# 10XGenomics/scan-rs

Hardware: AMD Instinct MI355X
Metric: cells/sec for top-50 PCA on 1000000x33000 @3% nnz; achieved HBM GB/s vs roofline (higher is better)
Workload: dtype f64

## Files before the change

### scan-rs_amd/csrc/dense.hip

```cpp
#include "common.hpp"

#include <algorithm>

namespace scanrs {

typedef double d2 __attribute__((ext_vector_type(2)));
typedef double d4 __attribute__((ext_vector_type(4)));

constexpr uint32_t DT = 128;
constexpr uint32_t DK = 16;
constexpr uint32_t DLD = 144;

__device__ __forceinline__ void tile_mma(const double *__restrict__ As, const double *__restrict__ Bs, uint32_t wi,
                                         uint32_t wj, uint32_t li, uint32_t lk, d4 (&acc)[4][4]) {
#pragma unroll
    for (uint32_t kk = 0; kk < DK / 4; kk++) {
        const uint32_t row = (kk * 4 + lk) * DLD;
        double a[4], b[4];
#pragma unroll
        for (int t = 0; t < 4; t++) {
            a[t] = As[row + wi * 64 + t * 16 + li];
            b[t] = Bs[row + wj * 64 + t * 16 + li];
        }
#pragma unroll
        for (int mi = 0; mi < 4; mi++)
#pragma unroll
            for (int nj = 0; nj < 4; nj++) acc[mi][nj] = __builtin_amdgcn_mfma_f64_16x16x4f64(a[mi], b[nj], acc[mi][nj], 0, 0, 0);
    }
}

__global__ __launch_bounds__(256) void gram_tiled_kernel(const double *__restrict__ X, uint32_t ldx, uint32_t n,
                                                         const double *__restrict__ Y, uint32_t ldy, uint32_t m, uint64_t rows,
                                                         uint64_t rows_per_split, const uint32_t *__restrict__ tile_ij,
                                                         double *__restrict__ slab, const int *__restrict__ skip) {
    if (skip && *skip) return;
    __shared__ double As[DK * DLD];
    __shared__ double Bs[DK * DLD];
    const uint32_t tid = threadIdx.x, lane = tid & 63u, w = tid >> 6;
    const uint32_t li = lane & 15u, lk = lane >> 4, wi = w >> 1, wj = w & 1u;
    const uint32_t i0 = tile_ij[2 * blockIdx.x] * DT, j0 = tile_ij[2 * blockIdx.x + 1] * DT;
    const uint64_t r0 = (uint64_t)blockIdx.y * rows_per_split;
    const uint64_t r1 = min(rows, r0 + rows_per_split);
    d4 acc[4][4];
#pragma unroll
    for (int a = 0; a < 4; a++)
#pragma unroll
        for (int b = 0; b < 4; b++) acc[a][b] = (d4){0, 0, 0, 0};
    const uint32_t sc = lane * 2u;
    d2 xa[4], yb[4];
    auto load_block = [&](uint64_t r) {
#pragma unroll
        for (int h = 0; h < 4; h++) {
            const uint64_t gr = r + w * 4u + h;
            const bool rv = gr < r1;
            const uint32_t c = sc;
            xa[h] = (d2){0.0, 0.0};
            yb[h] = (d2){0.0, 0.0};
            if (rv) {
                const double *xr = X + gr * ldx + i0 + c;
                const double *yr = Y + gr * ldy + j0 + c;
                if (i0 + c + 1 < n)
                    xa[h] = *reinterpret_cast<const d2 *>(xr);
                else if (i0 + c < n)
                    xa[h].x = xr[0];
                if (j0 + c + 1 < m)
                    yb[h] = *reinterpret_cast<const d2 *>(yr);
                else if (j0 + c < m)
                    yb[h].x = yr[0];
            }
        }
    };
    auto store_block = [&]() {
#pragma unroll
        for (int h = 0; h < 4; h++) {
            *reinterpret_cast<d2 *>(&As[(w * 4u + h) * DLD + sc]) = xa[h];
            *reinterpret_cast<d2 *>(&Bs[(w * 4u + h) * DLD + sc]) = yb[h];
        }
    };
    if (r0 < r1) {
        load_block(r0);
        store_block();
    }
    __syncthreads();
    for (uint64_t r = r0; r < r1; r += DK) {
        const bool more = r + DK < r1;
        if (more) load_block(r + DK);
        tile_mma(As, Bs, wi, wj, li, lk, acc);
        __syncthreads();
        if (more) store_block();
        __syncthreads();
    }
    double *__restrict__ dst = slab + (size_t)blockIdx.y * n * m;
#pragma unroll
    for (int mi = 0; mi < 4; mi++)
#pragma unroll
        for (int nj = 0; nj < 4; nj++)
#pragma unroll
            for (int reg = 0; reg < 4; reg++) {
                const uint32_t row = i0 + wi * 64 + mi * 16 + lk + 4 * reg;
                const uint32_t col = j0 + wj * 64 + nj * 16 + li;
                if (row < n && col < m) dst[(size_t)row * m + col] = acc[mi][nj][reg];
            }
}

__global__ void gram_tiled_finish_kernel(const double *__restrict__ slab, uint32_t splits, uint32_t n, uint32_t m,
                                         int symmetric, double *__restrict__ C, const int *__restrict__ skip) {
    if (skip && *skip) return;
    const uint64_t e = (uint64_t)blockIdx.x * blockDim.x + threadIdx.x;
    if (e >= (uint64_t)n * m) return;
    uint32_t row = (uint32_t)(e / m), col = (uint32_t)(e % m);
    uint64_t src = e;
    if (symmetric && row / DT > col / DT) src = (uint64_t)col * m + row;
    double s = 0.0;
    for (uint32_t k = 0; k < splits; k++) s += slab[(size_t)k * n * m + src];
    C[e] = s;
}

__global__ __launch_bounds__(256) void gemm_tiled_kernel(const double *__restrict__ X, uint32_t ldx, uint32_t n,
                                                         const double *__restrict__ W, uint32_t ldw, uint32_t m, uint64_t rows,
                                                         double alpha, double beta, const double *Cin, uint32_t ldc,
                                                         double *Out, uint32_t ldo, const int *__restrict__ skip) {
    if (skip && *skip) return;
    __shared__ double As[DK * DLD];
    __shared__ double Bs[DK * DLD];
    const uint32_t tid = threadIdx.x, lane = tid & 63u, w = tid >> 6;
    const uint32_t li = lane & 15u, lk = lane >> 4, wi = w >> 1, wj = w & 1u;
    const uint64_t r0 = (uint64_t)blockIdx.x * DT;
    const uint32_t j0 = blockIdx.y * DT;
    d4 acc[4][4];
#pragma unroll
    for (int a = 0; a < 4; a++)
#pragma unroll
        for (int b = 0; b < 4; b++) acc[a][b] = (d4){0, 0, 0, 0};
    const uint32_t ai = tid >> 3, ak = (tid & 7u) * 2u;
    const uint32_t bk = tid >> 4, bc = (tid & 15u) * 8u;
    d2 av[4], bv[4];
    auto load_block = [&](uint32_t k0) {
        const uint32_t kb = k0 + bk;
        const double *wr = W + (size_t)kb * ldw + j0 + bc;
        const uint32_t kk = k0 + ak;
#pragma unroll
        for (int h = 0; h < 4; h++) {
            const uint64_t arow = r0 + ai + 32u * h;
            av[h] = (d2){0.0, 0.0};
            if (arow < rows) {
                const double *xr = X + arow * ldx + kk;
                if (kk + 1 < n)
                    av[h] = *reinterpret_cast<const d2 *>(xr);
                else if (kk < n)
                    av[h].x = xr[0];
            }
            const uint32_t c = bc + 2u * h;
            bv[h] = (d2){0.0, 0.0};
            if (kb < n) {
                if (j0 + c + 1 < m)
                    bv[h].x = wr[2 * h], bv[h].y = wr[2 * h + 1];
                else if (j0 + c < m)
                    bv[h].x = wr[2 * h];
            }
        }
    };
    auto store_block = [&]() {
#pragma unroll
        for (int h = 0; h < 4; h++) {
            As[ak * DLD + ai + 32u * h] = av[h].x;
            As[(ak + 1u) * DLD + ai + 32u * h] = av[h].y;
            *reinterpret_cast<d2 *>(&Bs[bk * DLD + bc + 2u * h]) = bv[h];
        }
    };
    if (n > 0) {
        load_block(0);
        store_block();
    }
    __syncthreads();
    for (uint32_t k0 = 0; k0 < n; k0 += DK) {
        const bool more = k0 + DK < n;
        if (more) load_block(k0 + DK);
        tile_mma(As, Bs, wi, wj, li, lk, acc);
        __syncthreads();
        if (more) store_block();
        __syncthreads();
    }
#pragma unroll
    for (int mi = 0; mi < 4; mi++)
#pragma unroll
        for (int reg = 0; reg < 4; reg++) {
            const uint64_t row = r0 + wi * 64 + mi * 16 + lk + 4 * reg;
            if (row >= rows) continue;
#pragma unroll
            for (int nj = 0; nj < 4; nj++) {
                const uint32_t col = j0 + wj * 64 + nj * 16 + li;
                if (col >= m) continue;
                double r = alpha * acc[mi][nj][reg];
                if (beta != 0.0) r = fma(beta, Cin[row * ldc + col], r);
                Out[row * ldo + col] = r;
            }
        }
}

constexpr uint32_t SK_R = 256, SK_C = 64, SK_ALD = 272, SK_BLD = 80;
__global__ __launch_bounds__(256) void gemm_skinny_kernel(const double *__restrict__ X, uint32_t ldx, uint32_t n,
                                                          const double *__restrict__ W, uint32_t ldw, uint32_t m, uint64_t rows,
                                                          double alpha, double beta, const double *Cin, uint32_t ldc,
                                                          double *Out, uint32_t ldo, const int *__restrict__ skip) {
    if (skip && *skip) return;
    __shared__ double As[DK * SK_ALD];
    __shared__ double Bs[DK * SK_BLD];
    const uint32_t tid = threadIdx.x, lane = tid & 63u, w = tid >> 6;
    const uint32_t li = lane & 15u, lk = lane >> 4;
    const uint64_t r0 = (uint64_t)blockIdx.x * SK_R;
    const uint32_t j0 = blockIdx.y * SK_C;
    d4 acc[4][4];
#pragma unroll
    for (int a = 0; a < 4; a++)
#pragma unroll
        for (int b = 0; b < 4; b++) acc[a][b] = (d4){0, 0, 0, 0};
    const uint32_t ai = tid >> 3, ak = (tid & 7u) * 2u;
    const uint32_t bk = tid >> 4, bc = (tid & 15u) * 4u;
    d2 av[8];
    double bv[4];
    auto load_block = [&](uint32_t k0) {
        const uint32_t kk = k0 + ak;
#pragma unroll
        for (int h = 0; h < 8; h++) {
            const uint64_t arow = r0 + ai + 32u * h;
            av[h] = (d2){0.0, 0.0};
            if (arow < rows) {
                const double *xr = X + arow * ldx + kk;
                if (kk + 1 < n)
                    av[h] = *reinterpret_cast<const d2 *>(xr);
                else if (kk < n)
                    av[h].x = xr[0];
            }
        }
        const uint32_t kb = k0 + bk;
        const double *wr = W + (size_t)kb * ldw + j0 + bc;
#pragma unroll
        for (int h = 0; h < 4; h++) bv[h] = (kb < n && j0 + bc + h < m) ? wr[h] : 0.0;
    };
    auto store_block = [&]() {
#pragma unroll
        for (int h = 0; h < 8; h++) {
            As[ak * SK_ALD + ai + 32u * h] = av[h].x;
            As[(ak + 1u) * SK_ALD + ai + 32u * h] = av[h].y;
        }
#pragma unroll
        for (int h = 0; h < 4; h++) Bs[bk * SK_BLD + bc + h] = bv[h];
    };
    if (n > 0) {
        load_block(0);
        store_block();
    }
    __syncthreads();
    for (uint32_t k0 = 0; k0 < n; k0 += DK) {
        const bool more = k0 + DK < n;
        if (more) load_block(k0 + DK);
#pragma unroll
        for (uint32_t kk = 0; kk < DK / 4; kk++) {
            double a[4], b[4];
#pragma unroll
            for (int t = 0; t < 4; t++) {
                a[t] = As[(kk * 4 + lk) * SK_ALD + w * 64 + t * 16 + li];
                b[t] = Bs[(kk * 4 + lk) * SK_BLD + t * 16 + li];
            }
#pragma unroll
            for (int mi = 0; mi < 4; mi++)
#pragma unroll
                for (int nj = 0; nj < 4; nj++) acc[mi][nj] = __builtin_amdgcn_mfma_f64_16x16x4f64(a[mi], b[nj], acc[mi][nj], 0, 0, 0);
        }
        __syncthreads();
        if (more) store_block();
        __syncthreads();
    }
#pragma unroll
    for (int mi = 0; mi < 4; mi++)
#pragma unroll
        for (int reg = 0; reg < 4; reg++) {
            const uint64_t row = r0 + w * 64 + mi * 16 + lk + 4 * reg;
            if (row >= rows) continue;
#pragma unroll
            for (int nj = 0; nj < 4; nj++) {
                const uint32_t col = j0 + nj * 16 + li;
                if (col >= m) continue;
                double r = alpha * acc[mi][nj][reg];
                if (beta != 0.0) r = fma(beta, Cin[row * ldc + col], r);
                Out[row * ldo + col] = r;
            }
        }
}

constexpr uint32_t CHOL_NMAX = 128;
#ifndef SCANRS_CHOL_TD
#define SCANRS_CHOL_TD 32
#endif
constexpr uint32_t CHOL_TD = SCANRS_CHOL_TD;
constexpr int CHOL_E = CHOL_NMAX / CHOL_TD;
__global__ __launch_bounds__(CHOL_TD * CHOL_TD) void chol_rinv_kernel(const double *__restrict__ G, uint32_t n, double rows, int pass, int check_only,
                                                        int *__restrict__ ctl, double *__restrict__ Rinv, double *__restrict__ info) {
    __shared__ double rowbuf[CHOL_NMAX], colbuf[CHOL_NMAX], red[3 * CHOL_TD * CHOL_TD];
    const uint32_t tid = threadIdx.x, nt = blockDim.x, ty = tid / CHOL_TD, tx = tid % CHOL_TD;
    const uint32_t wy0 = (uint32_t)__builtin_amdgcn_readfirstlane((int)(tid >> 6)) * (64u / CHOL_TD);
    auto identity_out = [&]() {
        if (check_only) return;
        for (uint32_t e = tid; e < n * n; e += nt) Rinv[e] = (e / n == e % n) ? 1.0 : 0.0;
    };
    if (ctl[0]) {
        identity_out();
        return;
    }
    double err = 0.0, dmax = 0.0;
    int bad = 0;
    for (uint32_t e = tid; e < n * n; e += nt) {
        const uint32_t i = e / n, j = e - i * n;
        const double g = G[e];
        if (!isfinite(g)) bad = 1;
        err = fmax(err, fabs(g - (i == j ? 1.0 : 0.0)));
        if (i == j) dmax = fmax(dmax, g);
    }
    red[tid] = err;
    red[nt + tid] = dmax;
    red[2 * nt + tid] = (double)bad;
    __syncthreads();
    for (uint32_t s = nt / 2; s > 0; s >>= 1) {
        if (tid < s) {
            red[tid] = fmax(red[tid], red[tid + s]);
            red[nt + tid] = fmax(red[nt + tid], red[nt + tid + s]);
            red[2 * nt + tid] = fmax(red[2 * nt + tid], red[2 * nt + tid + s]);
        }
        __syncthreads();
    }
    err = red[0];
    dmax = red[nt];
    bad = red[2 * nt] != 0.0;
    __syncthreads();
    if (tid == 0 && info) info[0] = err;
    if (bad) {
        if (tid == 0) {
            ctl[0] = 1;
            ctl[1] = 2;
        }
        identity_out();
        return;
    }
    if (pass >= 1 && err < 5e-14 * sqrt((double)n)) {
        if (tid == 0) ctl[0] = 1;
        identity_out();
        return;
    }
    if (check_only) return;
    double A[CHOL_E][CHOL_E];
    double shift = 0.0;
    for (int tries = 0;; tries++) {
#pragma unroll
        for (int a = 0; a < CHOL_E; a++)
#pragma unroll
            for (int b = 0; b < CHOL_E; b++) {
                const uint32_t i = ty + CHOL_TD * a, j = tx + CHOL_TD * b;
                A[a][b] = (i < n && j < n && j >= i) ? G[i * n + j] + (i == j ? shift : 0.0) : 0.0;
            }
        bool failed = false;
        for (uint32_t k = 0; k < n; k++) {
            const uint32_t ka = k / CHOL_TD, kt = k % CHOL_TD;
#pragma unroll
            for (int a = 0; a < CHOL_E; a++)
                if ((uint32_t)a == ka && ty == kt) {
#pragma unroll
                    for (int b = 0; b < CHOL_E; b++) rowbuf[tx + CHOL_TD * b] = A[a][b];
                }
            __syncthreads();
            const double d = rowbuf[k];
            if (!(d > 0.0) || !isfinite(d)) {
                failed = true;
                break;
            }
            const double sq = sqrt(d), inv = 1.0 / sq;
            double g[CHOL_E], f[CHOL_E];
#pragma unroll
            for (int b = 0; b < CHOL_E; b++) g[b] = rowbuf[tx + CHOL_TD * b] * inv;
#pragma unroll
            for (int a = 0; a < CHOL_E; a++) f[a] = rowbuf[ty + CHOL_TD * a] * inv;
#pragma unroll
            for (int a = 0; a < CHOL_E; a++) {
                if (wy0 + 64u / CHOL_TD - 1u + CHOL_TD * a < k) continue;
                const uint32_t i = ty + CHOL_TD * a;
#pragma unroll
                for (int b = a; b < CHOL_E; b++) {
                    const uint32_t j = tx + CHOL_TD * b;
                    if (i == k)
                        A[a][b] = j == k ? sq : (j > k ? g[b] : 0.0);
                    else if (i > k && j >= i)
                        A[a][b] -= f[a] * g[b];
                }
            }
            __syncthreads();
        }
        __syncthreads();
        if (!failed) break;
        shift = shift == 0.0 ? 11.0 * (rows * n + (double)n * (n + 1)) * 1.1e-16 * dmax : shift * 100.0;
        if (tries + 1 > 12 || !(dmax > 0.0)) {
            if (tid == 0) {
                ctl[0] = 1;
                ctl[1] = 1;
            }
            identity_out();
            return;
        }
    }
    if (tid == 0 && info) info[1] = shift;
    for (int m = (int)n - 1; m >= 0; m--) {
        const uint32_t ma = (uint32_t)m / CHOL_TD, mt = (uint32_t)m % CHOL_TD;
#pragma unroll
        for (int b = 0; b < CHOL_E; b++)
            if ((uint32_t)b == ma && tx == mt) {
#pragma unroll
                for (int a = 0; a < CHOL_E; a++) colbuf[ty + CHOL_TD * a] = A[a][b];
            }
        __syncthreads();
        const double invd = 1.0 / colbuf[m];
#pragma unroll
        for (int a = 0; a < CHOL_E; a++)
            if ((uint32_t)a == ma && ty == mt) {
#pragma unroll
                for (int b = 0; b < CHOL_E; b++) {
                    const uint32_t j = tx + CHOL_TD * b;
                    const double x = j == (uint32_t)m ? invd : (j > (uint32_t)m ? -A[a][b] * invd : 0.0);
                    A[a][b] = x;
                    rowbuf[j] = x;
                }
            }
        __syncthreads();
        double cf[CHOL_E], xr[CHOL_E];
#pragma unroll
        for (int a = 0; a < CHOL_E; a++) cf[a] = colbuf[ty + CHOL_TD * a];
#pragma unroll
        for (int b = 0; b < CHOL_E; b++) xr[b] = rowbuf[tx + CHOL_TD * b];
#pragma unroll
        for (int a = 0; a < CHOL_E; a++) {
            if (wy0 + CHOL_TD * a >= (uint32_t)m) continue;
            const uint32_t k = ty + CHOL_TD * a;
#pragma unroll
            for (int b = a; b < CHOL_E; b++) {
                if (CHOL_TD * b + CHOL_TD - 1u < (uint32_t)m) continue;
                const uint32_t j = tx + CHOL_TD * b;
                if (k < (uint32_t)m && j >= (uint32_t)m) A[a][b] = j == (uint32_t)m ? cf[a] * xr[b] : fma(cf[a], xr[b], A[a][b]);
            }
        }
        __syncthreads();
    }
#pragma unroll
    for (int a = 0; a < CHOL_E; a++)
#pragma unroll
        for (int b = 0; b < CHOL_E; b++) {
            const uint32_t i = ty + CHOL_TD * a, j = tx + CHOL_TD * b;
            if (i < n && j < n) Rinv[i * n + j] = j >= i ? A[a][b] : 0.0;
        }
}

bool chol_rinv_ok(uint32_t n) { return n >= 1 && n <= CHOL_NMAX; }
void launch_chol_rinv(Storage &st, const double *G, uint32_t n, uint64_t rows, int pass, bool check_only, int *ctl, double *Rinv, double *info) {
    if (!chol_rinv_ok(n)) fail(SCANRS_ERR_ARGUMENT, "device Cholesky: n out of range");
    if (st.prof.on) st.prof.begin(st.stream, "chol_rinv", (double)n * n * 16.0);
    hipLaunchKernelGGL(chol_rinv_kernel, dim3(1), dim3(CHOL_TD * CHOL_TD), 0, st.stream, G, n, (double)rows, pass, check_only ? 1 : 0, ctl, Rinv, info);
    if (st.prof.on) st.prof.end(st.stream);
    SCANRS_HIP(hipGetLastError());
}

__global__ void absmax_flag_kernel(const double *__restrict__ C, uint32_t count, double limit, int *__restrict__ ctl, double *__restrict__ info) {
    __shared__ double red[256];
    double m = 0.0;
    for (uint32_t e = threadIdx.x; e < count; e += blockDim.x) {
        const double x = fabs(C[e]);
        m = (x > m || x != x) ? x : m;
    }
    red[threadIdx.x] = m;
    __syncthreads();
    for (uint32_t s = blockDim.x / 2; s > 0; s >>= 1) {
        if (threadIdx.x < s) {
            const double o = red[threadIdx.x + s];
            if (o > red[threadIdx.x] || o != o) red[threadIdx.x] = o;
        }
        __syncthreads();
    }
    if (threadIdx.x == 0) {
        if (info) info[0] = red[0];
        ctl[0] = 1;
        if (!(red[0] < limit) && ctl[1] == 0) ctl[1] = 3;
    }
}
void launch_absmax_flag(Storage &st, const double *C, uint32_t count, double limit, int *ctl, double *info) {
    hipLaunchKernelGGL(absmax_flag_kernel, dim3(1), dim3(256), 0, st.stream, C, count, limit, ctl, info);
    SCANRS_HIP(hipGetLastError());
}

bool gram_tiled_ok(uint32_t n, uint32_t m, uint64_t rows) { return n >= 48 && m >= 48 && rows >= 2048; }
bool gemm_tiled_ok(uint32_t n, uint32_t m, uint64_t rows) { return n >= 16 && m >= 48 && rows >= 2048; }

void launch_gram_tiled(Storage &st, const double *X, uint32_t ldx, uint32_t n, const double *Y, uint32_t ldy, uint32_t m,
                       uint64_t rows, double *C) {
    const uint32_t tn = (n + DT - 1) / DT, tm = (m + DT - 1) / DT;
    const bool symmetric = X == Y && ldx == ldy && n == m;
    std::vector<uint32_t> tiles;
    for (uint32_t i = 0; i < tn; i++)
        for (uint32_t j = symmetric ? i : 0; j < tm; j++) {
            tiles.push_back(i);
            tiles.push_back(j);
        }
    const uint32_t n_tiles = (uint32_t)tiles.size() / 2;
    char tkey[64];
    snprintf(tkey, sizeof tkey, "gramt_tiles_%u_%u_%d", tn, tm, symmetric ? 1 : 0);
    uint32_t *d_tiles = st.scratch.get<uint32_t>(tkey, tiles.size());
    if (st.scratch.filled.insert(tkey).second) {
        SCANRS_HIP(hipMemcpyAsync(d_tiles, tiles.data(), tiles.size() * 4, hipMemcpyHostToDevice, st.stream));
        SCANRS_SYNC(st.stream);
    }
    uint64_t splits = std::max<uint64_t>(1, std::min<uint64_t>((rows + 255) / 256, (2048 + n_tiles - 1) / n_tiles));
    uint64_t rps = (rows + splits - 1) / splits;
    rps = (rps + DK - 1) / DK * DK;
    splits = std::max<uint64_t>(1, (rows + rps - 1) / rps);
    double *slab = st.scratch.get<double>(st.skey("gram_slab"), (size_t)splits * n * m);
    if (st.prof.on) st.prof.begin(st.stream, "gram_tiled_mfma_f64", (double)rows * (n + (symmetric ? 0 : m)) * 8.0 + (double)n * m * 8.0);
    hipLaunchKernelGGL(gram_tiled_kernel, dim3(n_tiles, (unsigned)splits), dim3(256), 0, st.stream, X, ldx, n, Y, ldy, m, rows, rps,
                       d_tiles, slab, st.skip_flag);
    hipLaunchKernelGGL(gram_tiled_finish_kernel, dim3((unsigned)(((uint64_t)n * m + 255) / 256)), dim3(256), 0, st.stream, slab,
                       (uint32_t)splits, n, m, symmetric ? 1 : 0, C, st.skip_flag);
    if (st.prof.on) st.prof.end(st.stream);
    SCANRS_HIP(hipGetLastError());
}

#include "dense_skinny.inc"

bool gemm_direct_ok(const double *X, uint32_t ldx, uint32_t n, uint32_t m, uint64_t rows) {
    return m >= 1u && m <= 4096u && n >= 16u && rows >= 64u && ldx % 2u == 0 && (reinterpret_cast<uintptr_t>(X) & 15u) == 0;
}
void launch_gemm_direct(Storage &st, const double *X, uint32_t ldx, uint32_t n, const double *W, uint32_t ldw, uint32_t m, uint64_t rows,
                        double alpha, double beta, const double *Cin, uint32_t ldc, double *Out, uint32_t ldo) {
    const uint32_t n_pad = (n + 15u) / 16u * 16u, groups = m <= 112u ? 1u : (m + 63u) / 64u, nt = ((m + 15u) / 16u + groups - 1u) / groups,
                   m_pad = nt * 16u * groups;
    double *Wt = st.scratch.get<double>(st.skey("skinny_wt"), (size_t)n_pad * m_pad);
    if (st.prof.on) st.prof.begin(st.stream, "gemm_skinny_mfma_f64", (double)rows * (n + m) * 8.0 + (double)n * m * 8.0);
    hipLaunchKernelGGL(skinny_wt_kernel, dim3((n_pad * m_pad + 255u) / 256u), dim3(256), 0, st.stream, W, ldw, n, m, n_pad, m_pad, Wt, st.skip_flag);
    const dim3 grid((unsigned)((rows + 64u * SKD_MT - 1) / (64u * SKD_MT)), groups);
#define SCANRS_SKD_LAUNCH(NT)                                                                                                                 \
    hipLaunchKernelGGL(gemm_skinny_direct_kernel<NT>, grid, dim3(256), 0, st.stream, X, ldx, n, Wt, n_pad, m, rows, alpha, beta, Cin, ldc, Out, ldo, \
                       st.skip_flag)
    switch (nt) {
    case 1: SCANRS_SKD_LAUNCH(1); break;
    case 2: SCANRS_SKD_LAUNCH(2); break;
    case 3: SCANRS_SKD_LAUNCH(3); break;
    case 4: SCANRS_SKD_LAUNCH(4); break;
    case 5: SCANRS_SKD_LAUNCH(5); break;
    case 6: SCANRS_SKD_LAUNCH(6); break;
    default: SCANRS_SKD_LAUNCH(7); break;
    }
#undef SCANRS_SKD_LAUNCH
    if (st.prof.on) st.prof.end(st.stream);
    SCANRS_HIP(hipGetLastError());
}

void launch_gemm_tiled(Storage &st, const double *X, uint32_t ldx, uint32_t n, const double *W, uint32_t ldw, uint32_t m,
                       uint64_t rows, double alpha, double beta, const double *Cin, uint32_t ldc, double *Out, uint32_t ldo) {
    if ((m - 1u) % DT < SK_C) {
        if (st.prof.on) st.prof.begin(st.stream, "gemm_skinny_mfma_f64", (double)rows * (n + m) * 8.0 + (double)n * m * 8.0);
        hipLaunchKernelGGL(gemm_skinny_kernel, dim3((unsigned)((rows + SK_R - 1) / SK_R), (m + SK_C - 1) / SK_C), dim3(256), 0, st.stream, X,
                           ldx, n, W, ldw, m, rows, alpha, beta, Cin, ldc, Out, ldo, st.skip_flag);
        if (st.prof.on) st.prof.end(st.stream);
        SCANRS_HIP(hipGetLastError());
        return;
    }
    if (st.prof.on) st.prof.begin(st.stream, "gemm_tiled_mfma_f64", (double)rows * (n + m) * 8.0 + (double)n * m * 8.0);
    if (trace_on()) fprintf(stderr, "[scanrs trace] gemm_tiled rows=%llu n=%u m=%u ldx=%u ldw=%u beta=%g\n", (unsigned long long)rows, n, m, ldx, ldw, beta);
    hipLaunchKernelGGL(gemm_tiled_kernel, dim3((unsigned)((rows + DT - 1) / DT), (m + DT - 1) / DT), dim3(256), 0, st.stream, X, ldx,
                       n, W, ldw, m, rows, alpha, beta, Cin, ldc, Out, ldo, st.skip_flag);
    if (st.prof.on) st.prof.end(st.stream);
    SCANRS_HIP(hipGetLastError());
}

__global__ void warm_dense_kernel() {}
void warm_dense(hipStream_t s) { hipLaunchKernelGGL(warm_dense_kernel, dim3(1), dim3(64), 0, s); }

}
```

Before: 5.025 million.

## Use blocked Cholesky and blocked triangular inverse in single-block chol_rinv kernel

Replaces the column-by-column Cholesky factorisation and row-by-row R-inverse, which needed two barriers per column, with a 32x32 blocked algorithm. A single wave factors and inverts each diagonal block using lane broadcasts, and the off-diagonal panel solve and trailing update run as shared-memory GEMM-like loops. The Gram check now uses wave shuffles instead of a tree reduction over shared memory, and the first attempt reuses the loaded G. The goal is fewer workgroup barriers in this serial one-block kernel, at the cost of more code complexity and a hard-coded tile size of 32.

```diff
diff --git a/scan-rs_amd/csrc/dense.hip b/scan-rs_amd/csrc/dense.hip
--- a/scan-rs_amd/csrc/dense.hip
+++ b/scan-rs_amd/csrc/dense.hip
@@ -290,16 +290,178 @@
 }
 
 constexpr uint32_t CHOL_NMAX = 128;
-#ifndef SCANRS_CHOL_TD
-#define SCANRS_CHOL_TD 32
-#endif
-constexpr uint32_t CHOL_TD = SCANRS_CHOL_TD;
+constexpr uint32_t CHOL_TD = 32;
 constexpr int CHOL_E = CHOL_NMAX / CHOL_TD;
+constexpr uint32_t CHOL_BLK = CHOL_TD * CHOL_TD;
+static_assert(CHOL_TD == 32 && CHOL_E == 4, "chol_rinv_kernel: a wave is two rows of the thread grid, lanes 0..31 are a block's columns");
+
+__device__ __forceinline__ double chol_lane_bcast(double v, int lane) {
+    const int lo = __builtin_amdgcn_readlane(__double2loint(v), lane), hi = __builtin_amdgcn_readlane(__double2hiint(v), lane);
+    return __hiloint2double(hi, lo);
+}
+__device__ __forceinline__ void chol_wave_sync() {
+    __builtin_amdgcn_fence(__ATOMIC_RELEASE, "workgroup");
+    __builtin_amdgcn_wave_barrier();
+    __builtin_amdgcn_fence(__ATOMIC_ACQUIRE, "workgroup");
+}
+
+__device__ __forceinline__ bool chol_diag_wave(double *Dk, double *Xk, uint32_t m, uint32_t lane) {
+    uint32_t j = lane & 31u;
+    asm volatile("" : "+v"(j));
+    double c[CHOL_TD];
+#pragma unroll
+    for (int i = 0; i < (int)CHOL_TD; i++) c[i] = Dk[i * CHOL_TD + j];
+    double myinv = 0.0;
+    bool ok = true;
+#pragma unroll
+    for (int k = 0; k < (int)CHOL_TD; k++) {
+        if (ok && (uint32_t)k < m) {
+            const double d = chol_lane_bcast(c[k], k);
+            if (!(d > 0.0) || !isfinite(d)) {
+                ok = false;
+            } else {
+                const double sq = sqrt(d), inv = 1.0 / sq;
+                const double rk = j == (uint32_t)k ? sq : c[k] * inv;
+                c[k] = rk;
+                if (j == (uint32_t)k) myinv = inv;
+#pragma unroll
+                for (int i = k + 1; i < (int)CHOL_TD; i++)
+                {
+                    c[i] = fma(-chol_lane_bcast(rk, i), rk, c[i]);
+                    if ((i & 3) == 3) __builtin_amdgcn_sched_barrier(0);
+                }
+            }
+        }
+    }
+    if (!ok) return false;
+    if (lane < CHOL_TD) {
+#pragma unroll
+        for (int i = 0; i < (int)CHOL_TD; i++) Dk[i * CHOL_TD + j] = c[i];
+    }
+    chol_wave_sync();
+    double x[CHOL_TD];
+#pragma unroll
+    for (int i = (int)CHOL_TD - 1; i >= 0; i--) {
+        if ((uint32_t)i >= m) {
+            x[i] = 0.0;
+            continue;
+        }
+        const double invd = chol_lane_bcast(myinv, i);
+        double s = 0.0;
+#pragma unroll
+        for (int q = i + 1; q < (int)CHOL_TD; q++)
+            s = fma(Dk[i * CHOL_TD + q], x[q], s);
+        x[i] = j == (uint32_t)i ? invd : (j > (uint32_t)i ? -s * invd : 0.0);
+    }
+    if (lane < CHOL_TD) {
+#pragma unroll
+        for (int i = 0; i < (int)CHOL_TD; i++) Xk[i * CHOL_TD + j] = x[i];
+    }
+    return true;
+}
+
+template <int KB> __device__ __forceinline__ void chol_stage(const double (&A)[CHOL_E][CHOL_E], double *Dk, double (*Pk)[CHOL_BLK], uint32_t t, uint32_t nblk) {
+    Dk[t] = A[KB][KB];
+#pragma unroll
+    for (int b = KB + 1; b < CHOL_E; b++)
+        if ((uint32_t)b < nblk) Pk[b - 1][t] = A[KB][b];
+}
+template <int KB>
+__device__ __forceinline__ void chol_solve(double (&A)[CHOL_E][CHOL_E], double (&acc)[CHOL_E], const double *Xk, const double (*Pk)[CHOL_BLK], uint32_t t, uint32_t ty,
+                                           uint32_t tx, uint32_t mend, uint32_t nblk) {
+    A[KB][KB] = Xk[t];
+#pragma unroll
+    for (int b = 0; b < CHOL_E; b++) acc[b] = 0.0;
+#pragma unroll 2
+    for (uint32_t m = 0; m < mend; m++) {
+        const double xv = Xk[m * CHOL_TD + ty];
+#pragma unroll
+        for (int b = KB + 1; b < CHOL_E; b++)
+            if ((uint32_t)b < nblk) acc[b] = fma(xv, Pk[b - 1][m * CHOL_TD + tx], acc[b]);
+    }
+}
+template <int KB> __device__ __forceinline__ void chol_publish(double (&A)[CHOL_E][CHOL_E], const double (&acc)[CHOL_E], double (*Pk)[CHOL_BLK], uint32_t t, uint32_t nblk) {
+#pragma unroll
+    for (int b = KB + 1; b < CHOL_E; b++)
+        if ((uint32_t)b < nblk) {
+            A[KB][b] = acc[b];
+            Pk[b - 1][t] = acc[b];
+        }
+}
+template <int KB> __device__ __forceinline__ void chol_update(double (&A)[CHOL_E][CHOL_E], const double (*Pk)[CHOL_BLK], uint32_t ty, uint32_t tx, uint32_t nblk) {
+#pragma unroll 4
+    for (uint32_t k = 0; k < CHOL_TD; k++) {
+        double g[CHOL_E];
+#pragma unroll
+        for (int b = KB + 1; b < CHOL_E; b++)
+            if ((uint32_t)b < nblk) g[b] = Pk[b - 1][k * CHOL_TD + tx];
+#pragma unroll
+        for (int a = KB + 1; a < CHOL_E; a++)
+            if ((uint32_t)a < nblk) {
+                const double f = Pk[a - 1][k * CHOL_TD + ty];
+#pragma unroll
+                for (int b = a; b < CHOL_E; b++)
+                    if ((uint32_t)b < nblk) A[a][b] = fma(-f, g[b], A[a][b]);
+            }
+    }
+}
+template <int AR>
+__device__ __forceinline__ void chol_inv_row(double (&A)[CHOL_E][CHOL_E], double *Dk, double *Xk, double (*Pk)[CHOL_BLK], uint32_t t, uint32_t ty, uint32_t tx, uint32_t wy0,
+                                             uint32_t nblk) {
+    double T[CHOL_E];
+#pragma unroll
+    for (int b = 0; b < CHOL_E; b++) T[b] = 0.0;
+#pragma unroll
+    for (int c = AR + 1; c < CHOL_E; c++) {
+        if ((uint32_t)c >= nblk) break;
+        Dk[t] = A[AR][c];
+#pragma unroll
+        for (int b = c; b < CHOL_E; b++)
+            if ((uint32_t)b < nblk) Pk[b - 1][t] = A[c][b];
+        __syncthreads();
+#pragma unroll 4
+        for (uint32_t m = 0; m < CHOL_TD; m++) {
+            const double r = Dk[ty * CHOL_TD + m];
+#pragma unroll
+            for (int b = c; b < CHOL_E; b++)
+                if ((uint32_t)b < nblk) T[b] = fma(r, Pk[b - 1][m * CHOL_TD + tx], T[b]);
+        }
+        __syncthreads();
+    }
+    Xk[t] = A[AR][AR];
+#pragma unroll
+    for (int b = AR + 1; b < CHOL_E; b++)
+        if ((uint32_t)b < nblk) Pk[b - 1][t] = T[b];
+    __syncthreads();
+#pragma unroll
+    for (int b = AR + 1; b < CHOL_E; b++) T[b] = 0.0;
+#pragma unroll 2
+    for (uint32_t m = wy0; m < CHOL_TD; m++) {
+        const double xv = Xk[ty * CHOL_TD + m];
+#pragma unroll
+        for (int b = AR + 1; b < CHOL_E; b++)
+            if ((uint32_t)b < nblk) T[b] = fma(xv, Pk[b - 1][m * CHOL_TD + tx], T[b]);
+    }
+#pragma unroll
+    for (int b = AR + 1; b < CHOL_E; b++)
+        if ((uint32_t)b < nblk) A[AR][b] = -T[b];
+    __syncthreads();
+}
+#define CHOL_BY_BLOCK(idx, call)      \
+    switch (idx) {                    \
+    case 0: { constexpr int KB = 0; call; } break; \
+    case 1: { constexpr int KB = 1; call; } break; \
+    case 2: { constexpr int KB = 2; call; } break; \
+    default: { constexpr int KB = 3; call; } break; \
+    }
+
 __global__ __launch_bounds__(CHOL_TD * CHOL_TD) void chol_rinv_kernel(const double *__restrict__ G, uint32_t n, double rows, int pass, int check_only,
                                                         int *__restrict__ ctl, double *__restrict__ Rinv, double *__restrict__ info) {
-    __shared__ double rowbuf[CHOL_NMAX], colbuf[CHOL_NMAX], red[3 * CHOL_TD * CHOL_TD];
-    const uint32_t tid = threadIdx.x, nt = blockDim.x, ty = tid / CHOL_TD, tx = tid % CHOL_TD;
-    const uint32_t wy0 = (uint32_t)__builtin_amdgcn_readfirstlane((int)(tid >> 6)) * (64u / CHOL_TD);
+    __shared__ double Dk[CHOL_BLK], Xk[CHOL_BLK], Pk[CHOL_E - 1][CHOL_BLK], red[3][CHOL_BLK / 64];
+    __shared__ int sfail;
+    const uint32_t tid = threadIdx.x, nt = blockDim.x, ty = tid / CHOL_TD, tx = tid % CHOL_TD, lane = tid & 63u;
+    const uint32_t wave = (uint32_t)__builtin_amdgcn_readfirstlane((int)(tid >> 6)), wy0 = wave * 2u;
+    const uint32_t nblk = (n + CHOL_TD - 1u) / CHOL_TD;
     auto identity_out = [&]() {
         if (check_only) return;
         for (uint32_t e = tid; e < n * n; e += nt) Rinv[e] = (e / n == e % n) ? 1.0 : 0.0;
@@ -308,31 +470,41 @@
         identity_out();
         return;
     }
-    double err = 0.0, dmax = 0.0;
-    int bad = 0;
-    for (uint32_t e = tid; e < n * n; e += nt) {
-        const uint32_t i = e / n, j = e - i * n;
-        const double g = G[e];
-        if (!isfinite(g)) bad = 1;
-        err = fmax(err, fabs(g - (i == j ? 1.0 : 0.0)));
-        if (i == j) dmax = fmax(dmax, g);
-    }
-    red[tid] = err;
-    red[nt + tid] = dmax;
-    red[2 * nt + tid] = (double)bad;
+    double A[CHOL_E][CHOL_E];
+    double err = 0.0, dmax = 0.0, badf = 0.0;
+#pragma unroll
+    for (int a = 0; a < CHOL_E; a++)
+#pragma unroll
+        for (int b = 0; b < CHOL_E; b++) {
+            const uint32_t i = ty + CHOL_TD * a, j = tx + CHOL_TD * b;
+            double g = 0.0;
+            if (i < n && j < n) {
+                g = G[i * n + j];
+                if (!isfinite(g)) badf = 1.0;
+                err = fmax(err, fabs(g - (i == j ? 1.0 : 0.0)));
+                if (i == j) dmax = fmax(dmax, g);
+            }
+            A[a][b] = g;
+        }
+#pragma unroll
+    for (int off = 32; off > 0; off >>= 1) {
+        err = fmax(err, __shfl_xor(err, off));
+        dmax = fmax(dmax, __shfl_xor(dmax, off));
+        badf = fmax(badf, __shfl_xor(badf, off));
+    }
+    if (lane == 0) {
+        red[0][wave] = err;
+        red[1][wave] = dmax;
+        red[2][wave] = badf;
+    }
     __syncthreads();
-    for (uint32_t s = nt / 2; s > 0; s >>= 1) {
-        if (tid < s) {
-            red[tid] = fmax(red[tid], red[tid + s]);
-            red[nt + tid] = fmax(red[nt + tid], red[nt + tid + s]);
-            red[2 * nt + tid] = fmax(red[2 * nt + tid], red[2 * nt + tid + s]);
-        }
-        __syncthreads();
-    }
-    err = red[0];
-    dmax = red[nt];
-    bad = red[2 * nt] != 0.0;
-    __syncthreads();
+#pragma unroll
+    for (uint32_t w = 0; w < CHOL_BLK / 64; w++) {
+        err = fmax(err, red[0][w]);
+        dmax = fmax(dmax, red[1][w]);
+        badf = fmax(badf, red[2][w]);
+    }
+    const bool bad = badf != 0.0;
     if (tid == 0 && info) info[0] = err;
     if (bad) {
         if (tid == 0) {
@@ -348,7 +520,6 @@
         return;
     }
     if (check_only) return;
-    double A[CHOL_E][CHOL_E];
     double shift = 0.0;
     for (int tries = 0;; tries++) {
 #pragma unroll
@@ -356,45 +527,32 @@
 #pragma unroll
             for (int b = 0; b < CHOL_E; b++) {
                 const uint32_t i = ty + CHOL_TD * a, j = tx + CHOL_TD * b;
-                A[a][b] = (i < n && j < n && j >= i) ? G[i * n + j] + (i == j ? shift : 0.0) : 0.0;
+                const bool in = i < n && j < n && j >= i;
+                if (tries > 0 && in) A[a][b] = G[i * n + j];
+                A[a][b] = in ? A[a][b] + (i == j ? shift : 0.0) : 0.0;
             }
         bool failed = false;
-        for (uint32_t k = 0; k < n; k++) {
-            const uint32_t ka = k / CHOL_TD, kt = k % CHOL_TD;
-#pragma unroll
-            for (int a = 0; a < CHOL_E; a++)
-                if ((uint32_t)a == ka && ty == kt) {
-#pragma unroll
-                    for (int b = 0; b < CHOL_E; b++) rowbuf[tx + CHOL_TD * b] = A[a][b];
-                }
+        for (uint32_t kb = 0; kb < nblk; kb++) {
+            CHOL_BY_BLOCK(kb, chol_stage<KB>(A, Dk, Pk, tid, nblk));
             __syncthreads();
-            const double d = rowbuf[k];
-            if (!(d > 0.0) || !isfinite(d)) {
+            if (wave == 0) {
+                const uint32_t m = min(CHOL_TD, n - CHOL_TD * kb);
+                const bool ok = chol_diag_wave(Dk, Xk, m, lane);
+                if (lane == 0) sfail = ok ? 0 : 1;
+            }
+            __syncthreads();
+            if (sfail) {
                 failed = true;
                 break;
             }
-            const double sq = sqrt(d), inv = 1.0 / sq;
-            double g[CHOL_E], f[CHOL_E];
-#pragma unroll
-            for (int b = 0; b < CHOL_E; b++) g[b] = rowbuf[tx + CHOL_TD * b] * inv;
-#pragma unroll
-            for (int a = 0; a < CHOL_E; a++) f[a] = rowbuf[ty + CHOL_TD * a] * inv;
-#pragma unroll
-            for (int a = 0; a < CHOL_E; a++) {
-                if (wy0 + 64u / CHOL_TD - 1u + CHOL_TD * a < k) continue;
-                const uint32_t i = ty + CHOL_TD * a;
-#pragma unroll
-                for (int b = a; b < CHOL_E; b++) {
-                    const uint32_t j = tx + CHOL_TD * b;
-                    if (i == k)
-                        A[a][b] = j == k ? sq : (j > k ? g[b] : 0.0);
-                    else if (i > k && j >= i)
-                        A[a][b] -= f[a] * g[b];
-                }
-            }
+            double acc[CHOL_E];
+            CHOL_BY_BLOCK(kb, chol_solve<KB>(A, acc, Xk, Pk, tid, ty, tx, wy0 + 2u, nblk));
             __syncthreads();
-        }
-        __syncthreads();
+            CHOL_BY_BLOCK(kb, chol_publish<KB>(A, acc, Pk, tid, nblk));
+            __syncthreads();
+            CHOL_BY_BLOCK(kb, chol_update<KB>(A, Pk, ty, tx, nblk));
+            __syncthreads();
+        }
         if (!failed) break;
         shift = shift == 0.0 ? 11.0 * (rows * n + (double)n * (n + 1)) * 1.1e-16 * dmax : shift * 100.0;
         if (tries + 1 > 12 || !(dmax > 0.0)) {
@@ -407,46 +565,7 @@
         }
     }
     if (tid == 0 && info) info[1] = shift;
-    for (int m = (int)n - 1; m >= 0; m--) {
-        const uint32_t ma = (uint32_t)m / CHOL_TD, mt = (uint32_t)m % CHOL_TD;
-#pragma unroll
-        for (int b = 0; b < CHOL_E; b++)
-            if ((uint32_t)b == ma && tx == mt) {
-#pragma unroll
-                for (int a = 0; a < CHOL_E; a++) colbuf[ty + CHOL_TD * a] = A[a][b];
-            }
-        __syncthreads();
-        const double invd = 1.0 / colbuf[m];
-#pragma unroll
-        for (int a = 0; a < CHOL_E; a++)
-            if ((uint32_t)a == ma && ty == mt) {
-#pragma unroll
-                for (int b = 0; b < CHOL_E; b++) {
-                    const uint32_t j = tx + CHOL_TD * b;
-                    const double x = j == (uint32_t)m ? invd : (j > (uint32_t)m ? -A[a][b] * invd : 0.0);
-                    A[a][b] = x;
-                    rowbuf[j] = x;
-                }
-            }
-        __syncthreads();
-        double cf[CHOL_E], xr[CHOL_E];
-#pragma unroll
-        for (int a = 0; a < CHOL_E; a++) cf[a] = colbuf[ty + CHOL_TD * a];
-#pragma unroll
-        for (int b = 0; b < CHOL_E; b++) xr[b] = rowbuf[tx + CHOL_TD * b];
-#pragma unroll
-        for (int a = 0; a < CHOL_E; a++) {
-            if (wy0 + CHOL_TD * a >= (uint32_t)m) continue;
-            const uint32_t k = ty + CHOL_TD * a;
-#pragma unroll
-            for (int b = a; b < CHOL_E; b++) {
-                if (CHOL_TD * b + CHOL_TD - 1u < (uint32_t)m) continue;
-                const uint32_t j = tx + CHOL_TD * b;
-                if (k < (uint32_t)m && j >= (uint32_t)m) A[a][b] = j == (uint32_t)m ? cf[a] * xr[b] : fma(cf[a], xr[b], A[a][b]);
-            }
-        }
-        __syncthreads();
-    }
+    for (int ar = (int)nblk - 2; ar >= 0; ar--) { CHOL_BY_BLOCK(ar, chol_inv_row<KB>(A, Dk, Xk, Pk, tid, ty, tx, wy0, nblk)); }
 #pragma unroll
     for (int a = 0; a < CHOL_E; a++)
 #pragma unroll
@@ -455,6 +574,7 @@
             if (i < n && j < n) Rinv[i * n + j] = j >= i ? A[a][b] : 0.0;
         }
 }
+#undef CHOL_BY_BLOCK
 
 bool chol_rinv_ok(uint32_t n) { return n >= 1 && n <= CHOL_NMAX; }
 void launch_chol_rinv(Storage &st, const double *G, uint32_t n, uint64_t rows, int pass, bool check_only, int *ctl, double *Rinv, double *info) {
```

Result: slower. 4.928 million (-1.9%).
